# Gavinli-lgf/belief-planning

Measured on AMD Instinct MI355X. Metric: branch-MPC solves/sec (whole node), highway N=20 M=3 branches, batch 4096 egos, higher is better.
Workload: dtype f64; 1 GPU; highway BranchMPC_CVaR closed loop, N=20, NB=1, m=3 (T=64, U=61), 4096 egos per GPU; batch_per_gpu=4096, global_batch=4096, world_size=1, parallelism=ego-sharded dp1, loop=per step: k_env + solve launches

## Files before the change

### belief-planning_amd/csrc/bmpc_ipm.h

```cpp
#pragma once

#include <type_traits>

#include "bmpc_tree.h"
#include "bmpc_wave.h"

#ifndef BMPC_EQUIL
#define BMPC_EQUIL 1
#endif
#ifndef BMPC_EQUIL_ITERS
#define BMPC_EQUIL_ITERS 3
#endif
#ifndef BMPC_TS_POST_RB_MIN
#define BMPC_TS_POST_RB_MIN 8
#endif
#ifndef BMPC_TS_POST_RB
#define BMPC_TS_POST_RB 4
#endif
#ifndef BMPC_PAIR_REFINE
#define BMPC_PAIR_REFINE 1
#endif
#ifndef BMPC_BLK_WAVE_SUBST
#define BMPC_BLK_WAVE_SUBST 1
#endif
// ... 6 lines not shown
#ifndef BMPC_WAVE_LU_MIN1
#define BMPC_WAVE_LU_MIN1 32
#endif
#ifndef BMPC_SUBST_REG
#define BMPC_SUBST_REG 1
#endif
#ifndef BMPC_REFINE_CALLS
#define BMPC_REFINE_CALLS 1
#endif
#ifndef BMPC_FLAT_PAIR
#define BMPC_FLAT_PAIR 1
#endif
#ifndef BMPC_IPM_LEAN_PASSES
#define BMPC_IPM_LEAN_PASSES 1
#endif
#ifndef BMPC_PAIR_BACK
#define BMPC_PAIR_BACK 1
#endif
#ifndef BMPC_TS_UN
#define BMPC_TS_UN 2
#endif
#ifndef BMPC_TS_UN_AV
#define BMPC_TS_UN_AV 8
#endif
#ifndef BMPC_NITREF
#define BMPC_NITREF 1
#endif
#ifndef BMPC_NITREF_INIT
#define BMPC_NITREF_INIT 0
#endif
// ... 288 lines not shown
}

template <int UC, class X>
BMPC_HD void cone_a_regs(const ConeGroups& G, const gdouble* a, bool jconj, int off, int q, double (&av)[UC]) {
#pragma unroll
  for (int uu = 0; uu < UC; ++uu) {
    const int i = G.gl + uu * G.cg;
    const double t = a[off + (i < q ? i : 0)];
    av[uu] = (i < q ? ((jconj && i > 0) ? -1.0 : 1.0) : 0.0) * t;
  }
}

template <int UC, class X>
BMPC_HD double cone_row0(const X& ex, const ConeGroups& G, const double (&v)[UC]) {
  return ex.gsum(G.gl == 0 ? v[0] : 0.0, G.cg);
}

template <class X, class = void>
struct inline_g { static constexpr bool value = false; };
template <class X>
struct inline_g<X, decltype((void)X::kInlineG)> { static constexpr bool value = X::kInlineG; };
template <class X, int NX, int NU, int WM = 0>
BMPC_HD void apply_G(const X ex, const Ctx& C, const gdouble* zv, gdouble* out, const gdouble* r3h = nullptr,
                     gdouble* tr = nullptr);
template <class X, int NX, int NU, int WM>
BMPC_HD void apply_G_body(const X ex, const Ctx Cin, const gdouble* zv, gdouble* out, const gdouble* r3h,
                          gdouble* tr) {
  const Ctx C = Cin.uniform();
  CPlan& P = *C.P;
  if constexpr (WM > 0) {
    r3h = uniform_ptr(r3h);
    if (!cone_regs(ex, P)) {
      apply_G<X, NX, NU, 0>(ex, C, zv, tr);
      if (WM == 3) apply_W(ex, C, 1, tr, out);
      else apply_W(ex, C, 1, tr, out, 1.0, r3h, -1.0);
      if (WM == 2) apply_W(ex, C, 1, out, out);
      return;
    }
  }
  constexpr int UC = X::kConeRegRows;
  double qx[NX];
  ctx_qx<NX>(C, qx);
  BMPC_PROF(C.ws, *C.L, PROF_APPLYG);
  BMPC_COUNT(C.ws, *C.L, PROF_NAPPLYG);
  BMPC_TIC(t_glp);
  const auto t = topo_view(P, ex);
  const int Nc = P.Nc;
  const gdouble* dh = C.at(C.L->dh);
  const gdouble* dli = C.at(C.L->dli);
  auto lp = [&](int row, double g) {
    if constexpr (WM == 0) {
      return g;
    } else {
      const double w = dli[row];
      if (WM == 3) return w * g;
      const double h = w * g - r3h[row];
      return WM == 2 ? w * h : h;
    }
  };
  struct Two { double a, b; };
  lane_batch<4>(ex, 0, P.T * Nc, [&](int it) {
    const int k = it / Nc, c = it % Nc;
    const double S = zv[P.oS + it];
    const double on = t.x_u[k] >= 0 ? 1.0 : 0.0;
    const int cr = c > 0 ? c - 1 : 0;
    const double m0 = c == 0 ? 1.0 : 0.0;
    double v = -S;
#pragma unroll
    for (int j = 0; j < NX; ++j) {
      const double fd = dh[k * NX + j], fx = fxv(P, ex, cr, j);
// ... 106 lines not shown
          for (int s2 = 0; s2 < NX; ++s2) zs[u2][s2] = zv[b + s2];
        }
#pragma unroll
        for (int u2 = 0; u2 < UC / 2; ++u2) {
          const int i = G.gl + (h + u2) * G.cg;
          const double m = mid_val(i >= 1 && i <= nmid ? i - 1 : 0, zs[u2]);
          v[h + u2] = i >= q ? 0.0 : i == 0 ? f0 : i == q - 1 ? -f0 : m;
        }
      }
      cone_a_regs<UC, X>(G, vn, true, off, q, a);
      const double sc = 1.0 / (k >= 0 ? eta[kk] : 1.0);
      cone_W_regs<UC>(ex, G, a, v, f0, sc, y);
#pragma unroll
      for (int uu = 0; uu < UC; ++uu) {
        const int i = G.gl + uu * G.cg;
        if (WM != 3) y[uu] = (i < q ? 1.0 : 0.0) * (y[uu] - r3h[off + (i < q ? i : 0)]);
      }
      if constexpr (WM == 2) {
        const double y0 = cone_row0<UC>(ex, G, y);
        cone_W_regs<UC>(ex, G, a, y, y0, sc, v);
#pragma unroll
        for (int uu = 0; uu < UC; ++uu) {
          const int i = G.gl + uu * G.cg;
          if (i < q) out[off + i] = v[uu];
        }
      } else {
#pragma unroll
        for (int uu = 0; uu < UC; ++uu) {
          const int i = G.gl + uu * G.cg;
          if (i < q) out[off + i] = y[uu];
        }
      }
    }
  }
  BMPC_TOC(C.ws, *C.L, PROF_G_CONE, t_gcone);
  ex.sync();
}
template <class X, int NX, int NU, int WM>
BMPC_FN_APPLY_G void apply_G_call(const X ex, const Ctx Cin, const gdouble* zv, gdouble* out, const gdouble* r3h,
                                  gdouble* tr) {
  apply_G_body<X, NX, NU, WM>(ex, Cin, zv, out, r3h, tr);
}
template <class X, int NX, int NU, int WM>
BMPC_HD void apply_G(const X ex, const Ctx& C, const gdouble* zv, gdouble* out, const gdouble* r3h, gdouble* tr) {
  if constexpr (inline_g<X>::value) apply_G_body<X, NX, NU, WM>(ex, C, zv, out, r3h, tr);
  else apply_G_call<X, NX, NU, WM>(ex, C, zv, out, r3h, tr);
}

template <class X, int NX, int NU>
BMPC_FN_APPLY_GT void apply_GT(const X ex, const Ctx Cin, const gdouble* r, gdouble* out, const gdouble* add = nullptr) {
  const Ctx C = Cin.uniform();
  add = uniform_ptr(add);
  const double sa = add ? 1.0 : 0.0;
  const gdouble* ad = add ? add : r;
  double qx[NX];
  ctx_qx<NX>(C, qx);
  CPlan& P = *C.P;
  BMPC_PROF(C.ws, *C.L, PROF_APPLYGT);
  const auto t = topo_view(P, ex);
  const int Nc = P.Nc;
  const gdouble* boost = C.at(C.L->boost);
  const gdouble* dh = C.at(C.L->dh);
  const double Qs = P.desc.Qslack[1];
  for (int k = ex.lane; k < P.T; k += ex.nlanes) {
    double ax[NX], cx[NX], os[BMPC_MAX_FX + 1];
#pragma unroll
    for (int j = 0; j < NX; ++j) ax[j] = 0.0, cx[j] = 0.0;
    const bool term = t.x_u[k] < 0;
    double fS = 0.0;
// ... 12 lines not shown
    } else if (k == 0) {
      const int kr = P.ncones - 1;
      const int off = t.cone_off[kr], q = t.cone_q[kr];
      fS = Qs * (r[off] - r[off + q - 1]) * ebeta<X>(boost, P.ncones, kr);
    }
    double dhk[NX];
#pragma unroll
    for (int j = 0; j < NX; ++j) dhk[j] = dh[k * NX + j];
    for (int c = 0; c < Nc; ++c) {
      const double rv = r[P.rFx + k * Nc + c];
      if (!term)
#pragma unroll
        for (int j = 0; j < NX; ++j) ax[j] += (c == 0 ? -dhk[j] : fxv(P, ex, c - 1, j)) * rv;
      os[c] = -rv - r[P.rPos + k * Nc + c] + fS;
    }
    for (int c = 0; c < Nc; ++c) out[P.oS + k * Nc + c] = os[c] + sa * ad[P.oS + k * Nc + c];
#pragma unroll
    for (int j = 0; j < NX; ++j) out[P.oX + k * NX + j] = (kc >= 0 ? ax[j] + cx[j] : ax[j]) + sa * ad[P.oX + k * NX + j];
  }
  for (int u = ex.lane; u < P.U; u += ex.nlanes) {
    double au[NU];
#pragma unroll
    for (int j = 0; j < NU; ++j) au[j] = 0.0;
    for (int rr = 0; rr < P.nFu; ++rr) {
      const double rv = r[P.rFu + u * P.nFu + rr];
#pragma unroll
      for (int j = 0; j < NU; ++j) au[j] += P.desc.Fu[rr * NU + j] * rv;
    }
    const int kc = t.u_cone[u];
    if (kc >= 0) {
      const int off = t.cone_off[kc];
      const int c = t.cone_c[kc];
      const int base = c >= 0 ? 1 + P.N * NX + (u - t.br_ndu[c]) * NU : 1;
#pragma unroll
      for (int s2 = 0; s2 < NU; ++s2) {
        double v = 0.0;
#pragma unroll
        for (int rr = 0; rr < NU; ++rr) v += -2.0 * P.Wu[rr * NU + s2] * r[off + base + rr];
        au[s2] += v;
      }
    }
#pragma unroll
    for (int j = 0; j < NU; ++j) out[P.oU + u * NU + j] = au[j] + sa * ad[P.oU + u * NU + j];
  }
  for (int i = ex.lane; i < P.ng; i += ex.nlanes) {
    double v = 0.0;
    const int gi = i == P.ng - 1 ? P.oJ : P.oRho + i;
    if (gi < P.oSig) v = -r[P.rRisk + (gi - P.oRho)];
    else if (gi >= P.oMup && gi < P.oS) v = -r[P.rRisk + P.bdim + (gi - P.oMup)];
    for (int k = 0; k < P.ncones; ++k) {
      const int off = t.cone_off[k], q = t.cone_q[k], c = t.cone_c[k];
      double w = 0.0;
      if (c >= 0) {
        const int b = t.cone_b[k], ii = t.cone_i[k];
        if (gi == P.oSig + b) w += 1.0;
        if (gi == P.oMup + b + ii) w += 1.0;
        if (gi == P.oMum + b + ii) w -= 1.0;
        if (t.br_child0[c] >= 0 && gi == P.oRho + c) w += 1.0;
      } else {
        if (gi == P.oJ) w -= 1.0;
        if (gi == P.oRho) w += 1.0;
      }
      if (w != 0.0) v += w * (r[off] - r[off + q - 1]) * ebeta<X>(boost, P.ncones, k);
    }
    out[gi] = v + sa * ad[gi];
  }
  ex.sync();
}

template <class X, int NX, int NU>
BMPC_HD void apply_A(const X ex, const Ctx& C, const gdouble* zv, gdouble* out) {
  CPlan& P = *C.P;
  const auto t = topo_view(P, ex);
  const gdouble* Ad = C.at(C.L->Ad);
  const gdouble* Bd = C.at(C.L->Bd);
  struct V4 { double v[NX]; };
  lane_batch<2>(ex, 0, P.T, [&](int k) {
    const int su = t.x_srcu[k], sx = t.x_srcx[k];
    V4 o;
#pragma unroll
    for (int r = 0; r < NX; ++r) o.v[r] = zv[P.oX + k * NX + r];
    if (su >= 0) {
      double xs[NX], us[NU];
// ... 11 lines not shown
    }
    return o;
  }, [&](int k, const V4& o) {
#pragma unroll
    for (int r = 0; r < NX; ++r) out[k * NX + r] = o.v[r];
  });
  const gdouble* p = C.at(C.L->p);
  for (int b = ex.lane; b < P.bdim; b += ex.nlanes) {
    double v = zv[P.oRho + b] + zv[P.oSig + b];
    for (int i = 0; i < P.m; ++i) v -= p[b * P.m + i] / P.desc.ralpha * zv[P.oMum + b * P.m + i];
    out[P.T * NX + b] = v;
  }
  ex.sync();
}

template <class X, int NX, int NU>
BMPC_HD void apply_AT(const X ex, const Ctx& C, const gdouble* y, gdouble* out) {
  CPlan& P = *C.P;
  const auto t = topo_view(P, ex);
  const gdouble* Ad = C.at(C.L->Ad);
  const gdouble* Bd = C.at(C.L->Bd);
  for (int k = ex.lane; k < P.T; k += ex.nlanes) {
    double ax[NX], au[NU];
#pragma unroll
    for (int r = 0; r < NX; ++r) ax[r] = y[k * NX + r];
#pragma unroll
    for (int r = 0; r < NU; ++r) au[r] = 0.0;
    const int u = t.x_u[k];
    if (u >= 0) {
      double ys[NX];
#pragma unroll
      for (int r = 0; r < NX; ++r) ys[r] = 0.0;
      for (int e = t.succ_off[k]; e < t.succ_off[k + 1]; ++e) {
        const int c = t.succ[e];
#pragma unroll
        for (int r = 0; r < NX; ++r) ys[r] += y[c * NX + r];
      }
#pragma unroll
      for (int s2 = 0; s2 < NX; ++s2) {
        double v = 0.0;
#pragma unroll
        for (int r = 0; r < NX; ++r) v += Ad[u * NX * NX + r * NX + s2] * ys[r];
        ax[s2] -= v;
      }
#pragma unroll
      for (int s2 = 0; s2 < NU; ++s2) {
        double v = 0.0;
#pragma unroll
        for (int r = 0; r < NX; ++r) v += Bd[u * NX * NU + r * NU + s2] * ys[r];
        au[s2] -= v;
      }
#pragma unroll
      for (int s2 = 0; s2 < NU; ++s2) out[P.oU + u * NU + s2] = au[s2];
    }
#pragma unroll
    for (int r = 0; r < NX; ++r) out[P.oX + k * NX + r] = ax[r];
  }
  lane_batch(ex, P.oS, P.oJ, [&](int) { return 0.0; }, [&](int i, double v) { out[i] = v; });
  const gdouble* p = C.at(C.L->p);
  for (int i = ex.lane; i < P.ng; i += ex.nlanes) {
    const int gi = i == P.ng - 1 ? P.oJ : P.oRho + i;
    double v = 0.0;
    if (gi < P.oSig) v = y[P.T * NX + (gi - P.oRho)];
    else if (gi < P.oMup) v = y[P.T * NX + (gi - P.oSig)];
    else if (gi >= P.oMum && gi < P.oS) {
      const int j = gi - P.oMum, b = j / P.m, ii = j % P.m;
      v = -p[b * P.m + ii] / P.desc.ralpha * y[P.T * NX + b];
    }
    out[gi] = v;
  }
  ex.sync();
}

template <class X, int NX, int NU>
BMPC_HD void build_hb(const X ex, const Ctx& C, gdouble* h, gdouble* bv) {
  CPlan& P = *C.P;
  const auto t = topo_view(P, ex);
  const int Nc = P.Nc;
  const gdouble* h0 = C.at(C.L->h0);
  for (int it = ex.lane; it < P.T * Nc; it += ex.nlanes) {
    const int k = it / Nc, c = it % Nc;
    double v = 0.0;
    if (t.x_u[k] >= 0) v = c == 0 ? h0[k] : bxv(P, ex, c - 1);
    h[P.rFx + it] = v;
    h[P.rPos + it] = 0.0;
  }
  for (int it = ex.lane; it < P.U * P.nFu; it += ex.nlanes) h[P.rFu + it] = P.desc.bu[it % P.nFu];
// ... 1852 lines not shown
  if constexpr (BMPC_WAVE_LU && RowLanes<X>::value && (MultiWave<X>::value || !X::kCoupLds)) {
    if (ns <= 64 && (MultiWave<X>::value || ns >= BMPC_WAVE_LU_MIN1)) {
      double bad = 0.0;
      if (ex.lane < 64) bad = small_lu_wave(ex.lane, M, coup_vec(ex, P.lds_piv), ns) ? 0.0 : 1.0;
      ok = ex.max(bad) == 0.0;
    } else {
      ok = small_lu(ex, M, coup_vec(ex, P.lds_piv), ns);
    }
  } else {
    ok = small_lu(ex, M, coup_vec(ex, P.lds_piv), ns);
  }
  BMPC_TOC(C.ws, L, PROF_LU, t_lu);
  return ok;
}

template <class X, int NX, int NU, bool R3ZERO>
BMPC_HD void kkt_back(const X ex, const Ctx& C, const gdouble* tz, const gdouble* r2, const gdouble* r3h,
                      gdouble* dx, gdouble* dy, gdouble* dzh, bool fin);

template <class X, int NX, int NU, bool R3ZERO = false>
BMPC_HD void kkt_solve_once(const X ex, const Ctx Cin, const gdouble* r1, const gdouble* r2,
                            const gdouble* r3h, gdouble* dx, gdouble* dy, gdouble* dzh, bool tr_ready, bool fin) {
  const Ctx C = Cin.uniform();
  CPlan& P = *C.P;
  CLayout& L = *C.L;
  gdouble* ws = C.ws;
  gdouble* tr = ws + L.k_r0;
  gdouble* tz = ws + L.k_nv0;
  if constexpr (R3ZERO) {
    tz = const_cast<gdouble*>(r1);
  } else {
    if (!tr_ready) apply_W(ex, C, 1, r3h, tr);
    apply_GT<X, NX, NU>(ex, C, tr, tz, r1);
  }
  tree_solve<X, NX, NU>(ex, C, 1, tz, 0, r2, 0, dx, 0, dy, 0);
  kkt_back<X, NX, NU, R3ZERO>(ex, C, tz, r2, r3h, dx, dy, dzh, fin);
}

template <class X, int NX, int NU, bool R3ZERO>
BMPC_HD void kkt_back(const X ex, const Ctx& C, const gdouble* tz, const gdouble* r2, const gdouble* r3h,
                      gdouble* dx, gdouble* dy, gdouble* dzh, bool fin) {
  CPlan& P = *C.P;
  CLayout& L = *C.L;
  BMPC_PROF(C.ws, L, PROF_BACK);
  gdouble* ws = C.ws;
  gdouble* tr = ws + L.k_r0;
  const int ng = P.ng, nb = P.bdim, nc = P.ncones, ns = P.nsm;
  auto* b = coup_vec(ex, P.lds_rhs);
  const gdouble* eta = ws + L.eta;
  if (coup_supp_dots(P)) {
    const auto t = topo_view(P, ex);
    for (int k0 = 0; k0 < nc; k0 += 16) {
      double acc[16];
      cone_supp_gdx(ex, P, t, ws + L.gk, P.nv, dx, k0, acc);
      if (ex.lane == 0)
        for (int a = 0; a < 16 && k0 + a < nc; ++a) b[ng + nb + k0 + a] = 2.0 / (eta[k0 + a] * eta[k0 + a]) * acc[a];
// ... 8 lines not shown
    }
  }
  for (int i = ex.lane; i < ng + nb; i += ex.nlanes) b[i] = i < ng ? tz[gvar(P, i)] : r2[P.T * NX + i - ng];
  ex.sync();
  BMPC_TIC(t_lus);
  small_lu_solve(ex, coup_mem(ex, ws, L, P, P.lds_M), coup_vec(ex, P.lds_piv), b, ns);
  BMPC_TOC(C.ws, L, PROF_LUS, t_lus);
  const auto* bc = b + ng + nb;
  const gdouble* colk = ws + L.colk;
  const gdouble* colnu = ws + L.colnu;
  const int n1 = P.oRho, n2 = n1 + (P.oJ - P.oS), n3 = n2 + P.T * NX;
  auto row = [&](int t, int& i, bool& isx) {
    isx = t < n2;
    i = t < n1 ? t : t < n2 ? P.oS + (t - n1) : t - n2;
  };
  lane_batch(ex, 0, n3, [&](int t) {
    int i;
    bool isx;
    row(t, i, isx);
    const gdouble* col = isx ? colk : colnu;
    const size_t cs = isx ? (size_t)P.nv : (size_t)P.neq;
    const gdouble* src = isx ? dx : dy;
    double v = src[i];
    for (int k0 = 0; k0 < nc; k0 += 4) {
      double c4[4], b4[4];
#pragma unroll
      for (int a = 0; a < 4; ++a) {
        c4[a] = col[(size_t)(k0 + a < nc ? k0 + a : nc - 1) * cs + i];
        b4[a] = k0 + a < nc ? bc[k0 + a] : 0.0;
      }
#pragma unroll
      for (int a = 0; a < 4; ++a) v -= b4[a] * c4[a];
    }
    return v;
  }, [&](int t, double v) {
    int i;
    bool isx;
    row(t, i, isx);
    if (isx) dx[i] = v;
    else dy[i] = v;
  });
  for (int i = ex.lane; i < ng + nb; i += ex.nlanes) {
    if (i < ng) dx[gvar(P, i)] = b[i];
    else dy[P.T * NX + i - ng] = b[i];
  }
  ex.sync();
  if constexpr (R3ZERO) apply_G<X, NX, NU, 3>(ex, C, dx, dzh, r3h, tr);
  else if (fin) apply_G<X, NX, NU, 2>(ex, C, dx, dzh, r3h, tr);
  else apply_G<X, NX, NU, 1>(ex, C, dx, dzh, r3h, tr);
}

template <class X, int NX, int NU, bool R3ZERO = false>
BMPC_HD void kkt_back_pair(const X ex, const Ctx& C, const gdouble* tz1, const gdouble* r21, const gdouble* r3h1,
                           gdouble* dx1, gdouble* dy1, gdouble* dzh1, const gdouble* tz2, const gdouble* r22,
                           const gdouble* r3h2, gdouble* dx2, gdouble* dy2, gdouble* dzh2, bool fin) {
  CPlan& P = *C.P;
  CLayout& L = *C.L;
  BMPC_PROF(C.ws, L, PROF_BACK);
  gdouble* ws = C.ws;
  gdouble* tr = ws + L.k_r0;
  const int ng = P.ng, nb = P.bdim, nc = P.ncones, ns = P.nsm;
  auto* b1 = coup_vec(ex, P.lds_rhs);
  auto* b2 = coup_vec(ex, P.lds_rhs2);
  const gdouble* eta = ws + L.eta;
  if (coup_supp_dots(P)) {
    const auto t = topo_view(P, ex);
    for (int k0 = 0; k0 < nc; k0 += 16) {
      double acc1[16], acc2[16];
      cone_supp_gdx2(ex, P, t, ws + L.gk, P.nv, dx1, dx2, k0, acc1, acc2);
      if (ex.lane == 0)
// ... 35 lines not shown
  if (!both) {
    small_lu_solve(ex, coup_mem(ex, ws, L, P, P.lds_M), coup_vec(ex, P.lds_piv), b1, ns);
    small_lu_solve(ex, coup_mem(ex, ws, L, P, P.lds_M), coup_vec(ex, P.lds_piv), b2, ns);
  }
  BMPC_TOC(C.ws, L, PROF_LUS, t_lus);
  const auto* bc1 = b1 + ng + nb;
  const auto* bc2 = b2 + ng + nb;
  const gdouble* colk = ws + L.colk;
  const gdouble* colnu = ws + L.colnu;
  const int n1 = P.oRho, n2 = n1 + (P.oJ - P.oS), n3 = n2 + P.T * NX;
  auto row = [&](int t, int& i, bool& isx) {
    isx = t < n2;
    i = t < n1 ? t : t < n2 ? P.oS + (t - n1) : t - n2;
  };
  struct V2 { double a, b; };
  lane_batch<4>(ex, 0, n3, [&](int t) {
    int i;
    bool isx;
    row(t, i, isx);
    const gdouble* col = isx ? colk : colnu;
    const size_t cs = isx ? (size_t)P.nv : (size_t)P.neq;
    const gdouble* s1 = isx ? dx1 : dy1;
    const gdouble* s2 = isx ? dx2 : dy2;
    double v1 = s1[i], v2 = s2[i];
    for (int k0 = 0; k0 < nc; k0 += 4) {
      double c4[4], p4[4], q4[4];
#pragma unroll
      for (int a = 0; a < 4; ++a) {
        c4[a] = col[(size_t)(k0 + a < nc ? k0 + a : nc - 1) * cs + i];
        p4[a] = k0 + a < nc ? bc1[k0 + a] : 0.0;
        q4[a] = k0 + a < nc ? bc2[k0 + a] : 0.0;
      }
#pragma unroll
      for (int a = 0; a < 4; ++a) v1 -= p4[a] * c4[a];
#pragma unroll
      for (int a = 0; a < 4; ++a) v2 -= q4[a] * c4[a];
    }
    return V2{v1, v2};
  }, [&](int t, V2 v) {
    int i;
    bool isx;
    row(t, i, isx);
    if (isx) dx1[i] = v.a, dx2[i] = v.b;
    else dy1[i] = v.a, dy2[i] = v.b;
  });
  for (int i = ex.lane; i < ng + nb; i += ex.nlanes) {
    if (i < ng) dx1[gvar(P, i)] = b1[i], dx2[gvar(P, i)] = b2[i];
    else dy1[P.T * NX + i - ng] = b1[i], dy2[P.T * NX + i - ng] = b2[i];
  }
  ex.sync();
  if constexpr (R3ZERO) {
    apply_G<X, NX, NU, 3>(ex, C, dx1, dzh1, r3h1, tr);
    apply_G<X, NX, NU, 3>(ex, C, dx2, dzh2, r3h2, tr);
  } else if (fin) {
    apply_G<X, NX, NU, 2>(ex, C, dx1, dzh1, r3h1, tr);
    apply_G<X, NX, NU, 2>(ex, C, dx2, dzh2, r3h2, tr);
  } else {
    apply_G<X, NX, NU, 1>(ex, C, dx1, dzh1, r3h1, tr);
    apply_G<X, NX, NU, 1>(ex, C, dx2, dzh2, r3h2, tr);
  }
}

template <class X, int NX, int NU>
BMPC_HD void kkt_refine(const X ex, const Ctx& C, const gdouble* r1, const gdouble* r2, const gdouble* r3h,
                        gdouble* dx, gdouble* dy, gdouble* dz, int nitref);

// ... 22 lines not shown
  gdouble* ws = C.ws;
  gdouble* e1 = ws + L.k_e1;
  gdouble* e2 = ws + L.k_e2;
  gdouble* e3 = ws + L.k_e3;
  gdouble* cx = ws + L.k_cx;
  gdouble* cy = ws + L.k_cy;
  gdouble* cz = ws + L.k_cz;
  gdouble* tv = ws + L.k_nv1;
  double msc = nitref == 0 ? 0.0 : lane_extreme<8, 1>(ex, 0, P.nrows, [&](int i) { return fabs(r3h[i]); });
  double sc = 0.0, prev = 1e300;
  for (int itr = 0; itr < nitref; ++itr) {
#if defined(BMPC_PROFILE) && defined(__HIP_DEVICE_COMPILE__)
    ProfScope _pr(C.ws, L.prof, PROF_REFINE);
#endif
    double merr = -1e300;
    apply_W(ex, C, 1, dz, e3);
    apply_GT<X, NX, NU>(ex, C, e3, tv);
    apply_AT<X, NX, NU>(ex, C, dy, e1);
    lane_batch<16>(ex, 0, P.nv, [&](int i) { const double a = r1[i]; msc = fmax(msc, fabs(a)); return a - e1[i] - tv[i]; },
                   [&](int i, double v) { e1[i] = v; merr = fmax(merr, fabs(v)); });
    apply_A<X, NX, NU>(ex, C, dx, e2);
    lane_batch(ex, 0, P.neq, [&](int i) { const double a = r2[i]; msc = fmax(msc, fabs(a)); return a - e2[i]; },
               [&](int i, double v) { e2[i] = v; merr = fmax(merr, fabs(v)); });
    if (itr == 0) sc = ex.max(msc);
    const double err = ex.max(merr);
    ex.sync();
    BMPC_TRACE("   refine %d err %.3e sc %.3e\n", itr, err, sc);
    if (!(err > BMPC_REFTOL * fmax(sc, 1.0))) break;
    if (BMPC_REF_STALL > 0 && itr > 0) {
      if (ex.uniform(!(err < prev))) {
        lane_batch<16>(ex, 0, P.nv, [&](int i) { return dx[i] - cx[i]; }, [&](int i, double v) { dx[i] = v; });
        lane_batch(ex, 0, P.neq, [&](int i) { return dy[i] - cy[i]; }, [&](int i, double v) { dy[i] = v; });
        lane_batch<16>(ex, 0, P.nrows, [&](int i) { return dz[i] - cz[i]; }, [&](int i, double v) { dz[i] = v; });
        ex.sync();
        break;
      }
      if (ex.uniform(prev < BMPC_REF_STALL * err)) break;
    }
    prev = err;
    kkt_solve_once<X, NX, NU, true>(ex, C, e1, e2, nullptr, cx, cy, cz, false, false);
    lane_batch<16>(ex, 0, P.nv, [&](int i) { return dx[i] + cx[i]; }, [&](int i, double v) { dx[i] = v; });
    lane_batch(ex, 0, P.neq, [&](int i) { return dy[i] + cy[i]; }, [&](int i, double v) { dy[i] = v; });
    lane_batch<16>(ex, 0, P.nrows, [&](int i) { return dz[i] + cz[i]; }, [&](int i, double v) { dz[i] = v; });
    ex.sync();
  }
  apply_W(ex, C, 1, dz, dz);
}

#if BMPC_REFINE_CALLS
template <class X, int NX, int NU>
BMPC_FN void refine_back_pair(const X ex, const Ctx Cin) {
  const Ctx C = Cin.uniform();
  CPlan& P = *C.P;
  CLayout& L = *C.L;
  gdouble* ws = C.ws;
  const size_t nv = P.nv, neq = P.neq, nr = P.nrows;
  gdouble* cx = ws + L.k_cx;
  gdouble* cy = ws + L.k_cy;
  gdouble* cz = ws + L.k_cz;
  kkt_back_pair<X, NX, NU, true>(ex, C, ws + L.k_e1, ws + L.k_e2, nullptr, cx, cy, cz, ws + L.k_e1 + nv,
                                 ws + L.k_e2 + neq, nullptr, cx + nv, cy + neq, cz + nr, false);
}
template <class X, int NX, int NU>
BMPC_FN void refine_solve_one(const X ex, const Ctx Cin, int j) {
  const Ctx C = Cin.uniform();
  j = ex.uniform(j != 0) ? 1 : 0;
  CPlan& P = *C.P;
  CLayout& L = *C.L;
  gdouble* ws = C.ws;
  const size_t nv = P.nv, neq = P.neq, nr = P.nrows;
  kkt_solve_once<X, NX, NU, true>(ex, C, ws + L.k_e1 + j * nv, ws + L.k_e2 + j * neq, nullptr, ws + L.k_cx + j * nv,
                                  ws + L.k_cy + j * neq, ws + L.k_cz + j * nr, false, false);
}
#endif

template <class X, int NX, int NU>
BMPC_FN void kkt_refine_pair(const X ex, const Ctx Cin, const gdouble* r1a, const gdouble* r2a, const gdouble* r3ha,
                             gdouble* dxa, gdouble* dya, gdouble* dza, const gdouble* r1b, const gdouble* r2b,
                             const gdouble* r3hb, gdouble* dxb, gdouble* dyb, gdouble* dzb, int nitref) {
  const Ctx C = Cin.uniform();
  CPlan& P = *C.P;
  CLayout& L = *C.L;
  gdouble* ws = C.ws;
  const size_t nv = P.nv, neq = P.neq, nr = P.nrows;
  gdouble* e3 = ws + L.k_e3;
  gdouble* tv = ws + L.k_nv1;
  const gdouble* r1[2] = {r1a, r1b};
// ... 7 lines not shown
#pragma unroll
  for (int j = 0; j < 2; ++j)
    msc[j] = nitref == 0 ? 0.0 : lane_extreme<8, 1>(ex, 0, P.nrows, [&](int i) { return fabs(r3h[j][i]); });
  bool on[2] = {true, true};
  double prev[2] = {1e300, 1e300};
  for (int itr = 0; itr < nitref; ++itr) {
#if defined(BMPC_PROFILE) && defined(__HIP_DEVICE_COMPILE__)
    ProfScope _pr(C.ws, L.prof, PROF_REFINE);
#endif
#pragma unroll
    for (int j = 0; j < 2; ++j) {
      if (!ex.uniform(on[j])) continue;
      gdouble* e1 = ws + L.k_e1 + j * nv;
      gdouble* e2 = ws + L.k_e2 + j * neq;
      double merr = -1e300;
      apply_W(ex, C, 1, dz[j], e3);
      apply_GT<X, NX, NU>(ex, C, e3, tv);
      apply_AT<X, NX, NU>(ex, C, dy[j], e1);
      lane_batch<16>(ex, 0, P.nv, [&](int i) { const double a = r1[j][i]; msc[j] = fmax(msc[j], fabs(a)); return a - e1[i] - tv[i]; },
                     [&](int i, double v) { e1[i] = v; merr = fmax(merr, fabs(v)); });
      apply_A<X, NX, NU>(ex, C, dx[j], e2);
      lane_batch(ex, 0, P.neq, [&](int i) { const double a = r2[j][i]; msc[j] = fmax(msc[j], fabs(a)); return a - e2[i]; },
                 [&](int i, double v) { e2[i] = v; merr = fmax(merr, fabs(v)); });
      if (itr == 0) sc[j] = ex.max(msc[j]);
      const double err = ex.max(merr);
      ex.sync();
      on[j] = ex.uniform(err > BMPC_REFTOL * fmax(sc[j], 1.0));
      BMPC_TRACE("   refine[%d] %d err %.3e sc %.3e\n", j, itr, err, sc[j]);
      if (BMPC_REF_STALL > 0 && itr > 0 && on[j]) {
        if (ex.uniform(!(err < prev[j]))) {
          const gdouble* cxj = ws + L.k_cx + j * nv;
          const gdouble* cyj = ws + L.k_cy + j * neq;
          const gdouble* czj = ws + L.k_cz + j * nr;
          lane_batch<16>(ex, 0, P.nv, [&](int i) { return dx[j][i] - cxj[i]; }, [&](int i, double v) { dx[j][i] = v; });
          lane_batch(ex, 0, P.neq, [&](int i) { return dy[j][i] - cyj[i]; }, [&](int i, double v) { dy[j][i] = v; });
          lane_batch<16>(ex, 0, P.nrows, [&](int i) { return dz[j][i] - czj[i]; }, [&](int i, double v) { dz[j][i] = v; });
          ex.sync();
          on[j] = false;
        } else if (ex.uniform(prev[j] < BMPC_REF_STALL * err)) {
          on[j] = false;
        }
      }
      prev[j] = err;
    }
    if (!ex.uniform(on[0] || on[1])) break;
    gdouble* cx = ws + L.k_cx;
    gdouble* cy = ws + L.k_cy;
    gdouble* cz = ws + L.k_cz;
    if (ex.uniform(on[0] && on[1])) {
      tree_solve<X, NX, NU>(ex, C, 2, ws + L.k_e1, nv, ws + L.k_e2, neq, cx, nv, cy, neq);
#if BMPC_REFINE_CALLS
      refine_back_pair<X, NX, NU>(ex, C);
#else
      kkt_back_pair<X, NX, NU, true>(ex, C, ws + L.k_e1, ws + L.k_e2, nullptr, cx, cy, cz, ws + L.k_e1 + nv,
                                     ws + L.k_e2 + neq, nullptr, cx + nv, cy + neq, cz + nr, false);
#endif
    } else {
      const int j = on[0] ? 0 : 1;
#if BMPC_REFINE_CALLS
      refine_solve_one<X, NX, NU>(ex, C, j);
#else
      kkt_solve_once<X, NX, NU, true>(ex, C, ws + L.k_e1 + j * nv, ws + L.k_e2 + j * neq, nullptr, cx + j * nv,
                                      cy + j * neq, cz + j * nr, false, false);
#endif
    }
#pragma unroll
    for (int j = 0; j < 2; ++j) {
      if (!ex.uniform(on[j])) continue;
      const gdouble* cxj = cx + j * nv;
      const gdouble* cyj = cy + j * neq;
      const gdouble* czj = cz + j * nr;
      lane_batch<16>(ex, 0, P.nv, [&](int i) { return dx[j][i] + cxj[i]; }, [&](int i, double v) { dx[j][i] = v; });
      lane_batch(ex, 0, P.neq, [&](int i) { return dy[j][i] + cyj[i]; }, [&](int i, double v) { dy[j][i] = v; });
      lane_batch<16>(ex, 0, P.nrows, [&](int i) { return dz[j][i] + czj[i]; }, [&](int i, double v) { dz[j][i] = v; });
      ex.sync();
    }
  }
  apply_W(ex, C, 1, dza, dza);
  apply_W(ex, C, 1, dzb, dzb);
}

template <class X, int NX, int NU>
BMPC_FN bool kkt_solve_pair(const X ex, const Ctx Cin, const gdouble* r1c, const gdouble* r1a, const gdouble* r3a,
                            int nitref) {
  const Ctx C = Cin.uniform();
  r1c = uniform_ptr(r1c), r1a = uniform_ptr(r1a), r3a = uniform_ptr(r3a);
  CPlan& P = *C.P;
  CLayout& L = *C.L;
  BMPC_PROF(C.ws, L, PROF_KKT);
  gdouble* ws = C.ws;
  const size_t nv = P.nv, nc = P.ncones;
// ... 413 lines not shown
  BMPC_TOC(ws, L, PROF_INIT, t_init);
  double bs_pres = 0, bs_dres = 0, bs_relgap = 0, bs_gap = 0, bs_pcost = 0;
  bool bs_ok_cx = false;

  for (int it = 0; it <= P.desc.maxit; ++it) {
#if defined(BMPC_PROFILE) && defined(__HIP_DEVICE_COMPILE__)
    {
      BMPC_TIC(t_lat);
      const double probe = *(volatile const gdouble*)(ws + L.bestx + ex.lane);
      if (probe == 1.2345e300) ws[L.prof + PROF_STEP] += 0.0;
      BMPC_TOC(ws, L, PROF_STEP, t_lat);
    }
#endif
    BMPC_TIC(t_res);
    apply_AT<X, NX, NU>(ex, C, y, rx);
    apply_GT<X, NX, NU>(ex, C, z, tA);
    double acx[2] = {0.0, 0.0}, acy[3] = {0.0, 0.0, 0.0}, acz[5] = {0.0, 0.0, 0.0, 0.0, 0.0};
    struct R2b { double v, rs, xs; };
    lane_batch<8>(ex, 0, nv, [&](int i) {
      const double xi = x[i], q = BMPC_EQUIL ? xq[i] : 1.0;
      const double v = rx[i] + (tA[i] + (i == P.oJ ? tau : 0.0));
      return R2b{v, v / q, q * xi};
    }, [&](int i, R2b r) {
      rx[i] = r.v;
      if (BMPC_IPM_LEAN_PASSES) tA2[i] = -r.v;
      acx[0] += r.rs * r.rs;
      acx[1] += r.xs * r.xs;
    });
    apply_A<X, NX, NU>(ex, C, x, ry);
    struct R4 { double v, rs, a, ys; };
    lane_batch<8>(ex, 0, neq, [&](int i) {
      const double yi = y[i], bi = bv[i], q = BMPC_EQUIL ? aq[i] : 1.0;
      const double v = bi * tau - ry[i];
      return R4{v, v / q, bi * yi, q * yi};
    }, [&](int i, R4 r) { ry[i] = r.v; acy[0] += r.rs * r.rs; acy[1] += r.a; acy[2] += r.ys * r.ys; });
    apply_G<X, NX, NU>(ex, C, x, rz);
    struct R7 { double v, rs, a, zs, ss, sz; };
    lane_batch<4>(ex, 0, nr, [&](int i) {
      const double zi = z[i], si = s[i], hi = hv[i], q = BMPC_EQUIL ? gq[i] : 1.0;
// ... 210 lines not shown
```

Baseline: 75940 solves/s.

## Fuse residual subtraction and correction accumulation into operator apply passes

Adds fused variants of apply_GT, apply_AT and apply_G. They subtract the result from a source vector or accumulate it into an output inside the same pass, so separate elementwise lane_batch sweeps over nv/neq/nrows are no longer needed. This covers iterative refinement (residual computation and adding the dx/dy/dz corrections) and the main IPM residual computation. The aim is to cut global-memory traffic and sync passes per refinement step. The cost is more template variants, and a `rounded` asm barrier is used to keep the FP evaluation order unchanged, which can raise register pressure.

```diff
diff --git a/belief-planning_amd/csrc/bmpc_ipm.h b/belief-planning_amd/csrc/bmpc_ipm.h
--- a/belief-planning_amd/csrc/bmpc_ipm.h
+++ b/belief-planning_amd/csrc/bmpc_ipm.h
@@ -44,6 +44,19 @@
 #ifndef BMPC_IPM_LEAN_PASSES
 #define BMPC_IPM_LEAN_PASSES 1
 #endif
+#ifndef BMPC_IPM_FUSED_PASSES
+#define BMPC_IPM_FUSED_PASSES 1
+#endif
+#if !defined(__HIPCC__)
+#define BMPC_HOST_COUNT(ws, L, id) ((ws)[(L).prof + (id)] += 1.0)
+#else
+#define BMPC_HOST_COUNT(ws, L, id) ((void)0)
+#endif
+#define BMPC_REFC_SOLVE PROF_X1
+#define BMPC_REFC_PAIR PROF_X2
+#define BMPC_REFC_ONE_C PROF_X3
+#define BMPC_REFC_ONE_A PROF_X4
+#define BMPC_REFC_RES PROF_G_LP
 #ifndef BMPC_PAIR_BACK
 #define BMPC_PAIR_BACK 1
 #endif
@@ -362,6 +375,13 @@
 template <int UC, class X>
 BMPC_HD double cone_row0(const X& ex, const ConeGroups& G, const double (&v)[UC]) {
   return ex.gsum(G.gl == 0 ? v[0] : 0.0, G.cg);
+}
+
+BMPC_HD double rounded(double v) {
+#if defined(__HIP_DEVICE_COMPILE__)
+  asm("" : "+v"(v));
+#endif
+  return v;
 }
 
 template <class X, class = void>
@@ -380,6 +400,12 @@
     r3h = uniform_ptr(r3h);
     if (!cone_regs(ex, P)) {
       apply_G<X, NX, NU, 0>(ex, C, zv, tr);
+      if constexpr (WM == 4) {
+        apply_W(ex, C, 1, tr, tr);
+        lane_batch<16>(ex, 0, P.nrows, [&](int i) { return out[i] + tr[i]; }, [&](int i, double v) { out[i] = v; });
+        ex.sync();
+        return;
+      }
       if (WM == 3) apply_W(ex, C, 1, tr, out);
       else apply_W(ex, C, 1, tr, out, 1.0, r3h, -1.0);
       if (WM == 2) apply_W(ex, C, 1, out, out);
@@ -402,6 +428,7 @@
     } else {
       const double w = dli[row];
       if (WM == 3) return w * g;
+      if (WM == 4) return out[row] + rounded(w * g);
       const double h = w * g - r3h[row];
       return WM == 2 ? w * h : h;
     }
@@ -538,7 +565,7 @@
 #pragma unroll
       for (int uu = 0; uu < UC; ++uu) {
         const int i = G.gl + uu * G.cg;
-        if (WM != 3) y[uu] = (i < q ? 1.0 : 0.0) * (y[uu] - r3h[off + (i < q ? i : 0)]);
+        if (WM != 3 && WM != 4) y[uu] = (i < q ? 1.0 : 0.0) * (y[uu] - r3h[off + (i < q ? i : 0)]);
       }
       if constexpr (WM == 2) {
         const double y0 = cone_row0<UC>(ex, G, y);
@@ -547,6 +574,18 @@
         for (int uu = 0; uu < UC; ++uu) {
           const int i = G.gl + uu * G.cg;
           if (i < q) out[off + i] = v[uu];
+        }
+      } else if constexpr (WM == 4) {
+        double o[UC];
+#pragma unroll
+        for (int uu = 0; uu < UC; ++uu) {
+          const int i = G.gl + uu * G.cg;
+          o[uu] = out[off + (i < q ? i : 0)];
+        }
+#pragma unroll
+        for (int uu = 0; uu < UC; ++uu) {
+          const int i = G.gl + uu * G.cg;
+          if (i < q) out[off + i] = o[uu] + rounded(y[uu]);
         }
       } else {
 #pragma unroll
@@ -571,12 +610,24 @@
   else apply_G_call<X, NX, NU, WM>(ex, C, zv, out, r3h, tr);
 }
 
-template <class X, int NX, int NU>
-BMPC_FN_APPLY_GT void apply_GT(const X ex, const Ctx Cin, const gdouble* r, gdouble* out, const gdouble* add = nullptr) {
+template <class X, int NX, int NU, int AM>
+BMPC_HD double apply_GT_body(const X ex, const Ctx Cin, const gdouble* r, gdouble* out, const gdouble* add) {
   const Ctx C = Cin.uniform();
   add = uniform_ptr(add);
   const double sa = add ? 1.0 : 0.0;
   const gdouble* ad = add ? add : r;
+  double mx = -1e300;
+  auto put = [&](int i, double v) {
+    if constexpr (AM == 0) {
+      out[i] = v + sa * ad[i];
+    } else if constexpr (AM == 1) {
+      out[i] = i == C.P->oJ ? v : ad[i] + (v + 0.0);
+    } else {
+      const double e = ad[i] - rounded(v);
+      out[i] = e;
+      mx = fmax(mx, fabs(e));
+    }
+  };
   double qx[NX];
   ctx_qx<NX>(C, qx);
   CPlan& P = *C.P;
@@ -619,9 +670,9 @@
         for (int j = 0; j < NX; ++j) ax[j] += (c == 0 ? -dhk[j] : fxv(P, ex, c - 1, j)) * rv;
       os[c] = -rv - r[P.rPos + k * Nc + c] + fS;
     }
-    for (int c = 0; c < Nc; ++c) out[P.oS + k * Nc + c] = os[c] + sa * ad[P.oS + k * Nc + c];
-#pragma unroll
-    for (int j = 0; j < NX; ++j) out[P.oX + k * NX + j] = (kc >= 0 ? ax[j] + cx[j] : ax[j]) + sa * ad[P.oX + k * NX + j];
+    for (int c = 0; c < Nc; ++c) put(P.oS + k * Nc + c, os[c]);
+#pragma unroll
+    for (int j = 0; j < NX; ++j) put(P.oX + k * NX + j, kc >= 0 ? ax[j] + cx[j] : ax[j]);
   }
   for (int u = ex.lane; u < P.U; u += ex.nlanes) {
     double au[NU];
@@ -646,7 +697,7 @@
       }
     }
 #pragma unroll
-    for (int j = 0; j < NU; ++j) out[P.oU + u * NU + j] = au[j] + sa * ad[P.oU + u * NU + j];
+    for (int j = 0; j < NU; ++j) put(P.oU + u * NU + j, au[j]);
   }
   for (int i = ex.lane; i < P.ng; i += ex.nlanes) {
     double v = 0.0;
@@ -668,10 +719,25 @@
       }
       if (w != 0.0) v += w * (r[off] - r[off + q - 1]) * ebeta<X>(boost, P.ncones, k);
     }
-    out[gi] = v + sa * ad[gi];
+    put(gi, v);
   }
   ex.sync();
-}
+  return mx;
+}
+template <class X, int NX, int NU>
+BMPC_FN_APPLY_GT void apply_GT(const X ex, const Ctx Cin, const gdouble* r, gdouble* out, const gdouble* add = nullptr) {
+  apply_GT_body<X, NX, NU, 0>(ex, Cin, r, out, add);
+}
+#if BMPC_IPM_FUSED_PASSES
+template <class X, int NX, int NU>
+BMPC_FN_APPLY_GT void apply_GT_res(const X ex, const Ctx Cin, const gdouble* r, gdouble* out, const gdouble* add) {
+  apply_GT_body<X, NX, NU, 1>(ex, Cin, r, out, add);
+}
+template <class X, int NX, int NU>
+BMPC_FN_APPLY_GT double apply_GT_sub(const X ex, const Ctx Cin, const gdouble* r, gdouble* out, const gdouble* add) {
+  return apply_GT_body<X, NX, NU, 2>(ex, Cin, r, out, add);
+}
+#endif
 
 template <class X, int NX, int NU>
 BMPC_HD void apply_A(const X ex, const Ctx& C, const gdouble* zv, gdouble* out) {
@@ -713,19 +779,30 @@
   ex.sync();
 }
 
-template <class X, int NX, int NU>
-BMPC_HD void apply_AT(const X ex, const Ctx& C, const gdouble* y, gdouble* out) {
+template <class X, int NX, int NU, bool SUB = false>
+BMPC_HD void apply_AT(const X ex, const Ctx& C, const gdouble* y, gdouble* out, const gdouble* from = nullptr,
+                      double* msc = nullptr) {
   CPlan& P = *C.P;
   const auto t = topo_view(P, ex);
   const gdouble* Ad = C.at(C.L->Ad);
   const gdouble* Bd = C.at(C.L->Bd);
+  auto sub = [&](double a, double v) {
+    *msc = fmax(*msc, fabs(a));
+    return a - rounded(v);
+  };
   for (int k = ex.lane; k < P.T; k += ex.nlanes) {
-    double ax[NX], au[NU];
+    double ax[NX], au[NU], fx[NX], fu[NU];
 #pragma unroll
     for (int r = 0; r < NX; ++r) ax[r] = y[k * NX + r];
 #pragma unroll
     for (int r = 0; r < NU; ++r) au[r] = 0.0;
     const int u = t.x_u[k];
+    if constexpr (SUB) {
+#pragma unroll
+      for (int r = 0; r < NX; ++r) fx[r] = from[P.oX + k * NX + r];
+#pragma unroll
+      for (int r = 0; r < NU; ++r) fu[r] = from[P.oU + (u >= 0 ? u : 0) * NU + r];
+    }
     if (u >= 0) {
       double ys[NX];
 #pragma unroll
@@ -750,12 +827,21 @@
         au[s2] -= v;
       }
 #pragma unroll
-      for (int s2 = 0; s2 < NU; ++s2) out[P.oU + u * NU + s2] = au[s2];
-    }
-#pragma unroll
-    for (int r = 0; r < NX; ++r) out[P.oX + k * NX + r] = ax[r];
-  }
-  lane_batch(ex, P.oS, P.oJ, [&](int) { return 0.0; }, [&](int i, double v) { out[i] = v; });
+      for (int s2 = 0; s2 < NU; ++s2) {
+        if constexpr (SUB) out[P.oU + u * NU + s2] = sub(fu[s2], au[s2]);
+        else out[P.oU + u * NU + s2] = au[s2];
+      }
+    }
+#pragma unroll
+    for (int r = 0; r < NX; ++r) {
+      if constexpr (SUB) out[P.oX + k * NX + r] = sub(fx[r], ax[r]);
+      else out[P.oX + k * NX + r] = ax[r];
+    }
+  }
+  lane_batch(ex, P.oS, P.oJ, [&](int i) {
+    if constexpr (SUB) return sub(from[i], 0.0);
+    else return 0.0;
+  }, [&](int i, double v) { out[i] = v; });
   const gdouble* p = C.at(C.L->p);
   for (int i = ex.lane; i < P.ng; i += ex.nlanes) {
     const int gi = i == P.ng - 1 ? P.oJ : P.oRho + i;
@@ -766,10 +852,20 @@
       const int j = gi - P.oMum, b = j / P.m, ii = j % P.m;
       v = -p[b * P.m + ii] / P.desc.ralpha * y[P.T * NX + b];
     }
-    out[gi] = v;
+    if constexpr (SUB) out[gi] = sub(from[gi], v);
+    else out[gi] = v;
   }
   ex.sync();
 }
+
+#if BMPC_IPM_FUSED_PASSES
+template <class X, int NX, int NU>
+BMPC_FN double apply_AT_sub(const X ex, const Ctx Cin, const gdouble* y, gdouble* out, const gdouble* from, double msc) {
+  const Ctx C = Cin.uniform();
+  apply_AT<X, NX, NU, true>(ex, C, uniform_ptr(y), uniform_ptr(out), uniform_ptr(from), &msc);
+  return msc;
+}
+#endif
 
 template <class X, int NX, int NU>
 BMPC_HD void build_hb(const X ex, const Ctx& C, gdouble* h, gdouble* bv) {
@@ -2652,13 +2748,15 @@
   return ok;
 }
 
-template <class X, int NX, int NU, bool R3ZERO>
+template <class X, int NX, int NU, bool R3ZERO, bool ACC = false>
 BMPC_HD void kkt_back(const X ex, const Ctx& C, const gdouble* tz, const gdouble* r2, const gdouble* r3h,
-                      gdouble* dx, gdouble* dy, gdouble* dzh, bool fin);
-
-template <class X, int NX, int NU, bool R3ZERO = false>
+                      gdouble* dx, gdouble* dy, gdouble* dzh, bool fin, gdouble* ax = nullptr, gdouble* ay = nullptr,
+                      gdouble* azh = nullptr);
+
+template <class X, int NX, int NU, bool R3ZERO = false, bool ACC = false>
 BMPC_HD void kkt_solve_once(const X ex, const Ctx Cin, const gdouble* r1, const gdouble* r2,
-                            const gdouble* r3h, gdouble* dx, gdouble* dy, gdouble* dzh, bool tr_ready, bool fin) {
+                            const gdouble* r3h, gdouble* dx, gdouble* dy, gdouble* dzh, bool tr_ready, bool fin,
+                            gdouble* ax = nullptr, gdouble* ay = nullptr, gdouble* azh = nullptr) {
   const Ctx C = Cin.uniform();
   CPlan& P = *C.P;
   CLayout& L = *C.L;
@@ -2672,12 +2770,14 @@
     apply_GT<X, NX, NU>(ex, C, tr, tz, r1);
   }
   tree_solve<X, NX, NU>(ex, C, 1, tz, 0, r2, 0, dx, 0, dy, 0);
-  kkt_back<X, NX, NU, R3ZERO>(ex, C, tz, r2, r3h, dx, dy, dzh, fin);
-}
-
-template <class X, int NX, int NU, bool R3ZERO>
+  kkt_back<X, NX, NU, R3ZERO, ACC>(ex, C, tz, r2, r3h, dx, dy, dzh, fin, ax, ay, azh);
+}
+
+template <class X, int NX, int NU, bool R3ZERO, bool ACC>
 BMPC_HD void kkt_back(const X ex, const Ctx& C, const gdouble* tz, const gdouble* r2, const gdouble* r3h,
-                      gdouble* dx, gdouble* dy, gdouble* dzh, bool fin) {
+                      gdouble* dx, gdouble* dy, gdouble* dzh, bool fin, gdouble* ax, gdouble* ay, gdouble* azh) {
+  static_assert(!ACC || R3ZERO, "only a refinement correction is accumulated");
+  constexpr bool UNDO = BMPC_REF_STALL > 0;
   CPlan& P = *C.P;
   CLayout& L = *C.L;
   BMPC_PROF(C.ws, L, PROF_BACK);
@@ -2716,6 +2816,7 @@
     isx = t < n2;
     i = t < n1 ? t : t < n2 ? P.oS + (t - n1) : t - n2;
   };
+  struct VO { double v, o; };
   lane_batch(ex, 0, n3, [&](int t) {
     int i;
     bool isx;
@@ -2724,6 +2825,8 @@
     const size_t cs = isx ? (size_t)P.nv : (size_t)P.neq;
     const gdouble* src = isx ? dx : dy;
     double v = src[i];
+    double o = 0.0;
+    if constexpr (ACC) o = (isx ? ax : ay)[i];
     for (int k0 = 0; k0 < nc; k0 += 4) {
       double c4[4], b4[4];
 #pragma unroll
@@ -2734,28 +2837,50 @@
 #pragma unroll
       for (int a = 0; a < 4; ++a) v -= b4[a] * c4[a];
     }
-    return v;
-  }, [&](int t, double v) {
+    if constexpr (ACC) return VO{v, o + rounded(v)};
+    else return v;
+  }, [&](int t, auto r) {
     int i;
     bool isx;
     row(t, i, isx);
-    if (isx) dx[i] = v;
-    else dy[i] = v;
+    if constexpr (ACC) {
+      if (isx) dx[i] = r.v, ax[i] = r.o;
+      else {
+        if (UNDO) dy[i] = r.v;
+        ay[i] = r.o;
+      }
+    } else {
+      if (isx) dx[i] = r;
+      else dy[i] = r;
+    }
   });
   for (int i = ex.lane; i < ng + nb; i += ex.nlanes) {
     if (i < ng) dx[gvar(P, i)] = b[i];
-    else dy[P.T * NX + i - ng] = b[i];
+    else if (!ACC || UNDO) dy[P.T * NX + i - ng] = b[i];
+    if constexpr (ACC) {
+      if (i < ng) ax[gvar(P, i)] = ax[gvar(P, i)] + b[i];
+      else ay[P.T * NX + i - ng] = ay[P.T * NX + i - ng] + b[i];
+    }
   }
   ex.sync();
-  if constexpr (R3ZERO) apply_G<X, NX, NU, 3>(ex, C, dx, dzh, r3h, tr);
+  if constexpr (ACC) {
+    if (UNDO) apply_G<X, NX, NU, 3>(ex, C, dx, dzh, r3h, tr);
+    apply_G<X, NX, NU, 4>(ex, C, dx, azh, r3h, tr);
+  } else if constexpr (R3ZERO) apply_G<X, NX, NU, 3>(ex, C, dx, dzh, r3h, tr);
   else if (fin) apply_G<X, NX, NU, 2>(ex, C, dx, dzh, r3h, tr);
   else apply_G<X, NX, NU, 1>(ex, C, dx, dzh, r3h, tr);
 }
 
-template <class X, int NX, int NU, bool R3ZERO = false>
+template <class X, int NX, int NU, bool R3ZERO = false, bool ACC = false>
 BMPC_HD void kkt_back_pair(const X ex, const Ctx& C, const gdouble* tz1, const gdouble* r21, const gdouble* r3h1,
                            gdouble* dx1, gdouble* dy1, gdouble* dzh1, const gdouble* tz2, const gdouble* r22,
                            const gdouble* r3h2, gdouble* dx2, gdouble* dy2, gdouble* dzh2, bool fin) {
+  static_assert(!ACC || R3ZERO, "only refinement corrections are accumulated");
+  constexpr bool UNDO = BMPC_REF_STALL > 0;
+  gdouble* ax1 = C.ws + C.L->x1;
+  gdouble* ay1 = C.ws + C.L->y1;
+  gdouble* ax2 = C.ws + C.L->x2;
+  gdouble* ay2 = C.ws + C.L->y2;
   CPlan& P = *C.P;
   CLayout& L = *C.L;
   BMPC_PROF(C.ws, L, PROF_BACK);
@@ -2821,6 +2946,7 @@
     i = t < n1 ? t : t < n2 ? P.oS + (t - n1) : t - n2;
   };
   struct V2 { double a, b; };
+  struct V4 { double a, b, oa, ob; };
   lane_batch<4>(ex, 0, n3, [&](int t) {
     int i;
     bool isx;
@@ -2830,6 +2956,8 @@
     const gdouble* s1 = isx ? dx1 : dy1;
     const gdouble* s2 = isx ? dx2 : dy2;
     double v1 = s1[i], v2 = s2[i];
+    double o1 = 0.0, o2 = 0.0;
+    if constexpr (ACC) o1 = (isx ? ax1 : ay1)[i], o2 = (isx ? ax2 : ay2)[i];
     for (int k0 = 0; k0 < nc; k0 += 4) {
       double c4[4], p4[4], q4[4];
 #pragma unroll
@@ -2843,20 +2971,41 @@
 #pragma unroll
       for (int a = 0; a < 4; ++a) v2 -= q4[a] * c4[a];
     }
-    return V2{v1, v2};
-  }, [&](int t, V2 v) {
+    if constexpr (ACC) return V4{v1, v2, o1 + rounded(v1), o2 + rounded(v2)};
+    else return V2{v1, v2};
+  }, [&](int t, auto v) {
     int i;
     bool isx;
     row(t, i, isx);
     if (isx) dx1[i] = v.a, dx2[i] = v.b;
-    else dy1[i] = v.a, dy2[i] = v.b;
+    else if (!ACC || UNDO) dy1[i] = v.a, dy2[i] = v.b;
+    if constexpr (ACC) {
+      if (isx) ax1[i] = v.oa, ax2[i] = v.ob;
+      else ay1[i] = v.oa, ay2[i] = v.ob;
+    }
   });
   for (int i = ex.lane; i < ng + nb; i += ex.nlanes) {
     if (i < ng) dx1[gvar(P, i)] = b1[i], dx2[gvar(P, i)] = b2[i];
-    else dy1[P.T * NX + i - ng] = b1[i], dy2[P.T * NX + i - ng] = b2[i];
+    else if (!ACC || UNDO) dy1[P.T * NX + i - ng] = b1[i], dy2[P.T * NX + i - ng] = b2[i];
+    if constexpr (ACC) {
+      if (i < ng) {
+        ax1[gvar(P, i)] = ax1[gvar(P, i)] + b1[i];
+        ax2[gvar(P, i)] = ax2[gvar(P, i)] + b2[i];
+      } else {
+        ay1[P.T * NX + i - ng] = ay1[P.T * NX + i - ng] + b1[i];
+        ay2[P.T * NX + i - ng] = ay2[P.T * NX + i - ng] + b2[i];
+      }
+    }
   }
   ex.sync();
-  if constexpr (R3ZERO) {
+  if constexpr (ACC) {
+    if (UNDO) {
+      apply_G<X, NX, NU, 3>(ex, C, dx1, dzh1, r3h1, tr);
+      apply_G<X, NX, NU, 3>(ex, C, dx2, dzh2, r3h2, tr);
+    }
+    apply_G<X, NX, NU, 4>(ex, C, dx1, C.ws + C.L->z1, r3h1, tr);
+    apply_G<X, NX, NU, 4>(ex, C, dx2, C.ws + C.L->z2, r3h2, tr);
+  } else if constexpr (R3ZERO) {
     apply_G<X, NX, NU, 3>(ex, C, dx1, dzh1, r3h1, tr);
     apply_G<X, NX, NU, 3>(ex, C, dx2, dzh2, r3h2, tr);
   } else if (fin) {
@@ -2909,11 +3058,17 @@
     ProfScope _pr(C.ws, L.prof, PROF_REFINE);
 #endif
     double merr = -1e300;
+    BMPC_HOST_COUNT(ws, L, BMPC_REFC_RES);
     apply_W(ex, C, 1, dz, e3);
+#if BMPC_IPM_FUSED_PASSES
+    msc = apply_AT_sub<X, NX, NU>(ex, C, dy, e1, r1, msc);
+    merr = apply_GT_sub<X, NX, NU>(ex, C, e3, e1, e1);
+#else
     apply_GT<X, NX, NU>(ex, C, e3, tv);
     apply_AT<X, NX, NU>(ex, C, dy, e1);
     lane_batch<16>(ex, 0, P.nv, [&](int i) { const double a = r1[i]; msc = fmax(msc, fabs(a)); return a - e1[i] - tv[i]; },
                    [&](int i, double v) { e1[i] = v; merr = fmax(merr, fabs(v)); });
+#endif
     apply_A<X, NX, NU>(ex, C, dx, e2);
     lane_batch(ex, 0, P.neq, [&](int i) { const double a = r2[i]; msc = fmax(msc, fabs(a)); return a - e2[i]; },
                [&](int i, double v) { e2[i] = v; merr = fmax(merr, fabs(v)); });
@@ -2933,11 +3088,16 @@
       if (ex.uniform(prev < BMPC_REF_STALL * err)) break;
     }
     prev = err;
+    BMPC_HOST_COUNT(ws, L, BMPC_REFC_SOLVE);
+#if BMPC_IPM_FUSED_PASSES
+    kkt_solve_once<X, NX, NU, true, true>(ex, C, e1, e2, nullptr, cx, cy, cz, false, false, dx, dy, dz);
+#else
     kkt_solve_once<X, NX, NU, true>(ex, C, e1, e2, nullptr, cx, cy, cz, false, false);
     lane_batch<16>(ex, 0, P.nv, [&](int i) { return dx[i] + cx[i]; }, [&](int i, double v) { dx[i] = v; });
     lane_batch(ex, 0, P.neq, [&](int i) { return dy[i] + cy[i]; }, [&](int i, double v) { dy[i] = v; });
     lane_batch<16>(ex, 0, P.nrows, [&](int i) { return dz[i] + cz[i]; }, [&](int i, double v) { dz[i] = v; });
     ex.sync();
+#endif
   }
   apply_W(ex, C, 1, dz, dz);
 }
@@ -2953,8 +3113,9 @@
   gdouble* cx = ws + L.k_cx;
   gdouble* cy = ws + L.k_cy;
   gdouble* cz = ws + L.k_cz;
-  kkt_back_pair<X, NX, NU, true>(ex, C, ws + L.k_e1, ws + L.k_e2, nullptr, cx, cy, cz, ws + L.k_e1 + nv,
-                                 ws + L.k_e2 + neq, nullptr, cx + nv, cy + neq, cz + nr, false);
+  kkt_back_pair<X, NX, NU, true, BMPC_IPM_FUSED_PASSES != 0>(ex, C, ws + L.k_e1, ws + L.k_e2, nullptr, cx, cy, cz,
+                                                             ws + L.k_e1 + nv, ws + L.k_e2 + neq, nullptr, cx + nv,
+                                                             cy + neq, cz + nr, false);
 }
 template <class X, int NX, int NU>
 BMPC_FN void refine_solve_one(const X ex, const Ctx Cin, int j) {
@@ -2964,8 +3125,9 @@
   CLayout& L = *C.L;
   gdouble* ws = C.ws;
   const size_t nv = P.nv, neq = P.neq, nr = P.nrows;
-  kkt_solve_once<X, NX, NU, true>(ex, C, ws + L.k_e1 + j * nv, ws + L.k_e2 + j * neq, nullptr, ws + L.k_cx + j * nv,
-                                  ws + L.k_cy + j * neq, ws + L.k_cz + j * nr, false, false);
+  kkt_solve_once<X, NX, NU, true, BMPC_IPM_FUSED_PASSES != 0>(
+      ex, C, ws + L.k_e1 + j * nv, ws + L.k_e2 + j * neq, nullptr, ws + L.k_cx + j * nv, ws + L.k_cy + j * neq,
+      ws + L.k_cz + j * nr, false, false, ws + (j ? L.x2 : L.x1), ws + (j ? L.y2 : L.y1), ws + (j ? L.z2 : L.z1));
 }
 #endif
 
@@ -3003,11 +3165,17 @@
       gdouble* e1 = ws + L.k_e1 + j * nv;
       gdouble* e2 = ws + L.k_e2 + j * neq;
       double merr = -1e300;
+      BMPC_HOST_COUNT(ws, L, BMPC_REFC_RES);
       apply_W(ex, C, 1, dz[j], e3);
+#if BMPC_IPM_FUSED_PASSES
+      msc[j] = apply_AT_sub<X, NX, NU>(ex, C, dy[j], e1, r1[j], msc[j]);
+      merr = apply_GT_sub<X, NX, NU>(ex, C, e3, e1, e1);
+#else
       apply_GT<X, NX, NU>(ex, C, e3, tv);
       apply_AT<X, NX, NU>(ex, C, dy[j], e1);
       lane_batch<16>(ex, 0, P.nv, [&](int i) { const double a = r1[j][i]; msc[j] = fmax(msc[j], fabs(a)); return a - e1[i] - tv[i]; },
                      [&](int i, double v) { e1[i] = v; merr = fmax(merr, fabs(v)); });
+#endif
       apply_A<X, NX, NU>(ex, C, dx[j], e2);
       lane_batch(ex, 0, P.neq, [&](int i) { const double a = r2[j][i]; msc[j] = fmax(msc[j], fabs(a)); return a - e2[i]; },
                  [&](int i, double v) { e2[i] = v; merr = fmax(merr, fabs(v)); });
@@ -3037,22 +3205,27 @@
     gdouble* cy = ws + L.k_cy;
     gdouble* cz = ws + L.k_cz;
     if (ex.uniform(on[0] && on[1])) {
+      BMPC_HOST_COUNT(ws, L, BMPC_REFC_PAIR);
       tree_solve<X, NX, NU>(ex, C, 2, ws + L.k_e1, nv, ws + L.k_e2, neq, cx, nv, cy, neq);
 #if BMPC_REFINE_CALLS
       refine_back_pair<X, NX, NU>(ex, C);
 #else
-      kkt_back_pair<X, NX, NU, true>(ex, C, ws + L.k_e1, ws + L.k_e2, nullptr, cx, cy, cz, ws + L.k_e1 + nv,
-                                     ws + L.k_e2 + neq, nullptr, cx + nv, cy + neq, cz + nr, false);
+      kkt_back_pair<X, NX, NU, true, BMPC_IPM_FUSED_PASSES != 0>(ex, C, ws + L.k_e1, ws + L.k_e2, nullptr, cx, cy, cz,
+                                                                 ws + L.k_e1 + nv, ws + L.k_e2 + neq, nullptr, cx + nv,
+                                                                 cy + neq, cz + nr, false);
 #endif
     } else {
       const int j = on[0] ? 0 : 1;
+      BMPC_HOST_COUNT(ws, L, j ? BMPC_REFC_ONE_A : BMPC_REFC_ONE_C);
 #if BMPC_REFINE_CALLS
       refine_solve_one<X, NX, NU>(ex, C, j);
 #else
-      kkt_solve_once<X, NX, NU, true>(ex, C, ws + L.k_e1 + j * nv, ws + L.k_e2 + j * neq, nullptr, cx + j * nv,
-                                      cy + j * neq, cz + j * nr, false, false);
-#endif
-    }
+      kkt_solve_once<X, NX, NU, true, BMPC_IPM_FUSED_PASSES != 0>(
+          ex, C, ws + L.k_e1 + j * nv, ws + L.k_e2 + j * neq, nullptr, cx + j * nv, cy + j * neq, cz + j * nr, false,
+          false, dx[j], dy[j], dz[j]);
+#endif
+    }
+#if !BMPC_IPM_FUSED_PASSES
 #pragma unroll
     for (int j = 0; j < 2; ++j) {
       if (!ex.uniform(on[j])) continue;
@@ -3064,6 +3237,7 @@
       lane_batch<16>(ex, 0, P.nrows, [&](int i) { return dz[j][i] + czj[i]; }, [&](int i, double v) { dz[j][i] = v; });
       ex.sync();
     }
+#endif
   }
   apply_W(ex, C, 1, dza, dza);
   apply_W(ex, C, 1, dzb, dzb);
@@ -3507,15 +3681,24 @@
 #endif
     BMPC_TIC(t_res);
     apply_AT<X, NX, NU>(ex, C, y, rx);
+#if BMPC_IPM_FUSED_PASSES
+    apply_GT_res<X, NX, NU>(ex, C, z, rx, rx);
+#else
     apply_GT<X, NX, NU>(ex, C, z, tA);
+#endif
     double acx[2] = {0.0, 0.0}, acy[3] = {0.0, 0.0, 0.0}, acz[5] = {0.0, 0.0, 0.0, 0.0, 0.0};
     struct R2b { double v, rs, xs; };
     lane_batch<8>(ex, 0, nv, [&](int i) {
       const double xi = x[i], q = BMPC_EQUIL ? xq[i] : 1.0;
+#if BMPC_IPM_FUSED_PASSES
+      const double r0 = rx[i];
+      const double v = i == P.oJ ? 0.0 + (r0 + tau) : r0;
+#else
       const double v = rx[i] + (tA[i] + (i == P.oJ ? tau : 0.0));
+#endif
       return R2b{v, v / q, q * xi};
     }, [&](int i, R2b r) {
-      rx[i] = r.v;
+      if (!BMPC_IPM_FUSED_PASSES || i == P.oJ) rx[i] = r.v;
       if (BMPC_IPM_LEAN_PASSES) tA2[i] = -r.v;
       acx[0] += r.rs * r.rs;
       acx[1] += r.xs * r.xs;
```

Result: no change. 76220 solves/s (median of 6 runs) (+0.4%).
